# LuoweiZhou/VLP

Measured on NVIDIA H100. Metric: image_text_samples_per_sec, higher is better.
Workload: dtype bf16

## Files before the change

### include/vlpk.h

```cpp
#ifndef VLPK_H_
#define VLPK_H_

#include <stddef.h>
#include <stdint.h>

#ifdef __cplusplus
extern "C" {
#endif

#define VLPK_VERSION 102

#define VLPK_BF16 0
#define VLPK_F32 1
#define VLPK_I64 2
#define VLPK_MASK_ADDITIVE 0
#define VLPK_MASK_ZERO_ONE 1
#define VLPK_ACT_NONE 0
#define VLPK_ACT_RELU 1

typedef struct VlpkDropout {
  float p;
  uint64_t seed;
  const uint64_t* seed_dev;
} VlpkDropout;
// ... 105 lines not shown
                    int64_t k_bstride, const uint32_t* mask_bits, int mask_rows, int kv_slots, const float* lse, float* p, int64_t ld_p,
                    int64_t p_bstride, void* stream);

int vlpk_mha_fwd(const VlpkShape* s, const VlpkLayerWeights* w, const void* x, const void* x_kv, const uint32_t* mask_bits,
                 int mask_rows, VlpkLayerActs* a, float p_attn, float p_hidden, const VlpkDropout* drop, uint64_t layer_id,
                 void* stream);
int vlpk_ffn_fwd(const VlpkShape* s, const VlpkLayerWeights* w, VlpkLayerActs* a, float p_hidden, const VlpkDropout* drop,
                 uint64_t layer_id, void* stream);
int vlpk_layer_fwd(const VlpkShape* s, const VlpkLayerWeights* w, const void* x, const void* x_kv, const uint32_t* mask_bits,
                   int mask_rows, VlpkLayerActs* a, float p_attn, float p_hidden, const VlpkDropout* drop, uint64_t layer_id,
                   void* stream);
int vlpk_layer_bwd(const VlpkShape* s, const VlpkLayerWeights* w, const void* x, const uint32_t* mask_bits, int mask_rows,
                   const VlpkLayerActs* a, const void* dy, void* dx, const VlpkLayerGrads* g, const VlpkBwdScratch* ws,
                   float p_attn, float p_hidden, const VlpkDropout* drop, uint64_t layer_id, void* stream);

int vlpk_ffn_bwd(const VlpkShape* s, const VlpkLayerWeights* w, const VlpkLayerActs* a, const void* dy, void* dy1,
                 const VlpkLayerGrads* g, const VlpkBwdScratch* ws, float p_hidden, const VlpkDropout* drop, uint64_t layer_id,
                 void* stream);
int vlpk_mha_bwd(const VlpkShape* s, const VlpkLayerWeights* w, const void* x, const uint32_t* mask_bits, int mask_rows,
                 const VlpkLayerActs* a, const void* dy1, void* dx, const VlpkLayerGrads* g, const VlpkBwdScratch* ws, float p_attn,
                 float p_hidden, const VlpkDropout* drop, uint64_t layer_id, void* stream);
int vlpk_mha_incr_fwd(const VlpkShape* s, const VlpkLayerWeights* w, const void* x, const void* x_kv, const uint32_t* mask_bits,
                      int mask_rows, VlpkLayerActs* a, uint64_t layer_id, void* stream);
int vlpk_layer_cached_fwd(const VlpkShape* s, const VlpkLayerWeights* w, const void* x, void* kv_cache, int cache_rows, int pos,
                          const uint32_t* mask_bits, int mask_rows, VlpkLayerActs* a, uint64_t layer_id, void* stream);
int vlpk_layer_cached_group_fwd(const VlpkShape* s, const VlpkLayerWeights* w, const void* x, const void* prefix, int prefix_rows, int P,
                                void* text, int T, const int32_t* slots, int G, int pos, const uint32_t* mask_bits, int mask_rows,
                                VlpkLayerActs* a, uint64_t layer_id, void* stream);
int vlpk_workspace_bytes(const VlpkShape* s, size_t* out3);

int vlpk_encoder_fwd(const VlpkShape* s, int n_layers, const VlpkLayerWeights* w, const void* x, const uint32_t* mask_bits,
                     int mask_rows, VlpkLayerActs* acts, float p_attn, float p_hidden, const VlpkDropout* drop, void* stream);
int vlpk_encoder_bwd(const VlpkShape* s, int n_layers, const VlpkLayerWeights* w, const void* x, const uint32_t* mask_bits,
                     int mask_rows, const VlpkLayerActs* acts, const void* const* dys, void* dx0, const VlpkLayerGrads* grads,
                     const VlpkBwdScratch* ws, float p_attn, float p_hidden, const VlpkDropout* drop, void* stream);

int vlpk_decoder_ce_fwd(int R, int V, int H, const void* h, const void* w, const void* bias_pad, const int64_t* labels, void* logits,
                        float* lse, float* loss, void* stream);
int vlpk_decoder_ce_bwd(int R, int V, int H, const void* h, const void* w, const int64_t* labels, const void* logits, const float* lse,
                        const float* dloss, void* dlogits, float* dh, void* dw, float* dbias, void* stream);
int vlpk_decoder_ce_ls_fwd(int R, int V, int H, float eps, const void* h, const void* w, const void* bias_pad, const int64_t* labels,
                           void* logits, float* lse, float* loss, void* stream);
int vlpk_decoder_ce_ls_bwd(int R, int V, int H, float eps, const void* h, const void* w, const int64_t* labels, const void* logits,
                           const float* lse, const float* dloss, void* dlogits, float* dh, void* dw, float* dbias, void* stream);

typedef struct VlpkAdamTensor {
  void* param;
  const void* grad;
  float* master;
  float* m;
  float* v;
  int64_t n;
  float weight_decay;
  int32_t param_dtype;
  int32_t grad_dtype;
  int32_t reserved;
} VlpkAdamTensor;

int vlpk_bertadam_chunk(void);
int vlpk_bertadam_step(const VlpkAdamTensor* tensors_host, const VlpkAdamTensor* tensors_dev, const int32_t* chunk_prefix_host,
                       const int32_t* chunk_prefix_dev, int n_tensors, float* sqnorm_dev, double lr_scheduled, double b1, double b2,
                       double eps, double max_grad_norm, void* stream);

void vlpk_profile_enable(int on);
void vlpk_profile_reset(void);
int vlpk_profile_get(int cat, double* ms, double* work, int64_t* launches);
int64_t vlpk_launch_count(void);

int vlpk_beam_ngram_block(int rows, int K, int f, int T_cap, int n, const int32_t* hist_in, int32_t* hist_out, const int64_t* ptr,
                          const int64_t* wid, const int32_t* ignore, int n_ignore, float* logp, int64_t ld, int V, void* stream);

int vlpk_sample_tokens(int rows, int V, const void* logits, int64_t ld, const void* bias, int fp32, int mode, int topk, float topp,
                       uint64_t seed, int f, int64_t* seq, int T_cap, float* score, int32_t* finished, int32_t* live, int eos_id, int pad_id,
                       int block_eos, int n, const int32_t* ignore, int n_ignore, void* stream);

int vlpk_f32_to_bf16(const float* src, void* dst, int64_t n, void* stream);
int vlpk_colsum(const void* x, int64_t ld, int64_t M, int N, float* out, void* stream);
int vlpk_debug_dropout_mask(const VlpkDropout* drop, uint64_t site, int64_t n, unsigned char* out, void* stream);
int vlpk_add_bf16(void* dst, const void* a, const void* b, int64_t n, void* stream);

int vlpk_gemm(int M, int N, int K, int a_mn, const void* A, int64_t lda, int b_mn, const void* B, int64_t ldb, const void* bias,
              void* D0, int64_t ldd0, void* D1, int64_t ldd1, const void* aux, int64_t ld_aux, int epi, int splits, int bn,
              void* stream);

#ifdef __cplusplus
}
#endif
#endif
```

### vlp_b200/_lib.py

```python
import ctypes as C
import os

import torch

_HERE = os.path.dirname(os.path.abspath(__file__))
LIB_PATH = os.path.join(_HERE, "libvlpk.so")

c_void_p, c_int, c_i64, c_u64, c_float = C.c_void_p, C.c_int, C.c_int64, C.c_uint64, C.c_float


class VlpkDropout(C.Structure):
    _fields_ = [("p", c_float), ("seed", c_u64), ("seed_dev", c_void_p)]


class VlpkShape(C.Structure):
    _fields_ = [("B", C.c_int32), ("Lq", C.c_int32), ("Lkv", C.c_int32), ("H", C.c_int32), ("heads", C.c_int32),
                ("I", C.c_int32), ("kv_slots", C.c_int32)]


WEIGHT_FIELDS = ["wq", "wk", "wv", "bq", "bk", "bv", "wo", "bo", "ln1_g", "ln1_b", "w1", "b1", "w2", "b2", "ln2_g", "ln2_b"]
GRAD_FIELDS = ["wqkv", "bqkv", "wo", "bo", "ln1_g", "ln1_b", "w1", "b1", "w2", "b2", "ln2_g", "ln2_b"]
ACT_FIELDS = ["qkv", "ctx", "t1", "y1", "u", "hmid", "t2", "y", "lse", "stats1", "stats2", "kv", "drop_attn"]
SCRATCH_FIELDS = ["dz2", "dt2", "du", "dy1", "dz1", "dt1", "dctx", "dqkv", "dx"]

# ... 14 lines not shown
    _fields_ = [(n, c_void_p) for n in SCRATCH_FIELDS]


class VlpkAdamTensor(C.Structure):
    _fields_ = [("param", c_void_p), ("grad", c_void_p), ("master", c_void_p), ("m", c_void_p), ("v", c_void_p), ("n", c_i64),
                ("weight_decay", c_float), ("param_dtype", C.c_int32), ("grad_dtype", C.c_int32), ("reserved", C.c_int32)]


_P = c_void_p
_SIGS = {
    "vlpk_version": (c_int, []),
    "vlpk_last_error": (C.c_char_p, []),
    "vlpk_debug_set_option": (c_int, [C.c_char_p, c_int]),
    "vlpk_set_reserved_sms": (None, [c_int]),
    "vlpk_set_deterministic": (None, [c_int]),
    "vlpk_debug_plan_gemm": (c_int, [c_int] * 10 + [C.POINTER(c_int)]),
    "vlpk_mask_pack": (c_int, [_P, c_int, c_int, c_int, c_int, c_int, c_i64, c_i64, _P, _P]),
    "vlpk_mask_synth": (c_int, [_P, _P, c_int, c_int, c_int, _P, _P]),
    "vlpk_linear_fwd": (c_int, [c_int, c_int, c_int, _P, c_i64, _P, c_i64, _P, _P, c_i64, c_int, C.POINTER(VlpkDropout), c_u64, _P]),
    "vlpk_linear_bwd": (c_int, [c_int, c_int, c_int, _P, c_i64, _P, c_i64, _P, c_i64, _P, c_i64, _P, _P, c_i64, _P, c_i64, _P,
                                c_int, c_float, _P]),
    "vlpk_embed_fwd": (c_int, [c_int, c_int, c_int, c_int, c_int, _P, _P, _P, _P, _P, _P, _P, _P, _P, _P, _P, _P,
                               C.POINTER(VlpkDropout), c_u64, _P]),
    "vlpk_embed_bwd": (c_int, [c_int, c_int, c_int, c_int, c_int, _P, _P, _P, _P, _P, _P, _P, _P, _P, _P, _P, _P, _P, _P,
                               C.POINTER(VlpkDropout), c_u64, _P]),
    "vlpk_embed_tables_bwd": (c_int, [c_int, c_int, c_int, c_int, c_int, _P, _P, _P, _P, c_int, c_int, c_int, _P, _P, _P, _P, _P]),
    "vlpk_ln_res_drop_fwd": (c_int, [c_i64, c_int, _P, _P, _P, _P, _P, _P, C.POINTER(VlpkDropout), c_u64, _P]),
    "vlpk_ln_res_drop_bwd": (c_int, [c_i64, c_int, _P, _P, _P, _P, _P, _P, _P, _P, _P, _P, C.POINTER(VlpkDropout), c_u64, _P]),
    "vlpk_attn_core_fwd": (c_int, [c_int, c_int, c_int, c_int, _P, c_i64, _P, _P, c_i64, _P, c_int, _P, c_i64, _P,
                                   C.POINTER(VlpkDropout), c_u64, _P]),
    "vlpk_attn_core_bwd": (c_int, [c_int, c_int, c_int, _P, _P, _P, c_i64, _P, c_int, _P, _P, c_i64, _P, _P, _P, _P, c_i64,
                                   C.POINTER(VlpkDropout), c_u64, _P]),
    "vlpk_attn_core_fwd_wide": (c_int, [c_int, c_int, c_int, c_int, _P, c_i64, _P, _P, c_i64, _P, c_int, _P, c_i64, _P,
                                        C.POINTER(VlpkDropout), c_u64, c_int, _P]),
    "vlpk_attn_core_bwd_wide": (c_int, [c_int, c_int, c_int, _P, _P, _P, c_i64, _P, c_int, _P, _P, c_i64, _P, _P, _P, _P, c_i64,
                                        C.POINTER(VlpkDropout), c_u64, c_int, _P]),
    "vlpk_attn_probs": (c_int, [c_int, c_int, c_int, c_int, c_int, _P, c_i64, c_i64, _P, c_i64, c_i64, _P, c_int, c_int, _P, _P, c_i64,
                                c_i64, _P]),
    "vlpk_mha_fwd": (c_int, [C.POINTER(VlpkShape), C.POINTER(VlpkLayerWeights), _P, _P, _P, c_int, C.POINTER(VlpkLayerActs),
                             c_float, c_float, C.POINTER(VlpkDropout), c_u64, _P]),
    "vlpk_ffn_fwd": (c_int, [C.POINTER(VlpkShape), C.POINTER(VlpkLayerWeights), C.POINTER(VlpkLayerActs), c_float,
                             C.POINTER(VlpkDropout), c_u64, _P]),
    "vlpk_layer_fwd": (c_int, [C.POINTER(VlpkShape), C.POINTER(VlpkLayerWeights), _P, _P, _P, c_int, C.POINTER(VlpkLayerActs),
                               c_float, c_float, C.POINTER(VlpkDropout), c_u64, _P]),
    "vlpk_layer_bwd": (c_int, [C.POINTER(VlpkShape), C.POINTER(VlpkLayerWeights), _P, _P, c_int, C.POINTER(VlpkLayerActs), _P, _P,
                               C.POINTER(VlpkLayerGrads), C.POINTER(VlpkBwdScratch), c_float, c_float, C.POINTER(VlpkDropout),
                               c_u64, _P]),
    "vlpk_ffn_bwd": (c_int, [C.POINTER(VlpkShape), C.POINTER(VlpkLayerWeights), C.POINTER(VlpkLayerActs), _P, _P,
                             C.POINTER(VlpkLayerGrads), C.POINTER(VlpkBwdScratch), c_float, C.POINTER(VlpkDropout), c_u64, _P]),
    "vlpk_mha_bwd": (c_int, [C.POINTER(VlpkShape), C.POINTER(VlpkLayerWeights), _P, _P, c_int, C.POINTER(VlpkLayerActs), _P, _P,
                             C.POINTER(VlpkLayerGrads), C.POINTER(VlpkBwdScratch), c_float, c_float, C.POINTER(VlpkDropout),
                             c_u64, _P]),
    "vlpk_mha_incr_fwd": (c_int, [C.POINTER(VlpkShape), C.POINTER(VlpkLayerWeights), _P, _P, _P, c_int,
                                  C.POINTER(VlpkLayerActs), c_u64, _P]),
    "vlpk_layer_cached_fwd": (c_int, [C.POINTER(VlpkShape), C.POINTER(VlpkLayerWeights), _P, _P, c_int, c_int, _P, c_int,
                                      C.POINTER(VlpkLayerActs), c_u64, _P]),
    "vlpk_layer_cached_group_fwd": (c_int, [C.POINTER(VlpkShape), C.POINTER(VlpkLayerWeights), _P, _P, c_int, c_int, _P, c_int, _P, c_int,
                                            c_int, _P, c_int, C.POINTER(VlpkLayerActs), c_u64, _P]),
    "vlpk_workspace_bytes": (c_int, [C.POINTER(VlpkShape), C.POINTER(C.c_size_t)]),
    "vlpk_encoder_fwd": (c_int, [C.POINTER(VlpkShape), c_int, C.POINTER(VlpkLayerWeights), _P, _P, c_int,
                                 C.POINTER(VlpkLayerActs), c_float, c_float, C.POINTER(VlpkDropout), _P]),
    "vlpk_encoder_bwd": (c_int, [C.POINTER(VlpkShape), c_int, C.POINTER(VlpkLayerWeights), _P, _P, c_int,
                                 C.POINTER(VlpkLayerActs), C.POINTER(c_void_p), _P, C.POINTER(VlpkLayerGrads),
                                 C.POINTER(VlpkBwdScratch), c_float, c_float, C.POINTER(VlpkDropout), _P]),
    "vlpk_decoder_ce_fwd": (c_int, [c_int, c_int, c_int, _P, _P, _P, _P, _P, _P, _P, _P]),
    "vlpk_decoder_ce_bwd": (c_int, [c_int, c_int, c_int, _P, _P, _P, _P, _P, _P, _P, _P, _P, _P, _P]),
    "vlpk_decoder_ce_ls_fwd": (c_int, [c_int, c_int, c_int, c_float, _P, _P, _P, _P, _P, _P, _P, _P]),
    "vlpk_decoder_ce_ls_bwd": (c_int, [c_int, c_int, c_int, c_float, _P, _P, _P, _P, _P, _P, _P, _P, _P, _P, _P]),
    "vlpk_bertadam_chunk": (c_int, []),
    "vlpk_bertadam_step": (c_int, [_P, _P, _P, _P, c_int, _P, C.c_double, C.c_double, C.c_double, C.c_double, C.c_double, _P]),
    "vlpk_profile_enable": (None, [c_int]),
    "vlpk_profile_reset": (None, []),
    "vlpk_profile_get": (c_int, [c_int, C.POINTER(C.c_double), C.POINTER(C.c_double), C.POINTER(c_i64)]),
    "vlpk_launch_count": (c_i64, []),
    "vlpk_beam_ngram_block": (c_int, [c_int, c_int, c_int, c_int, c_int, _P, _P, _P, _P, _P, c_int, _P, c_i64, c_int, _P]),
    "vlpk_sample_tokens": (c_int, [c_int, c_int, _P, c_i64, _P, c_int, c_int, c_int, c_float, c_u64, c_int, _P, c_int, _P, _P, _P, c_int,
                                   c_int, c_int, c_int, _P, c_int, _P]),
    "vlpk_f32_to_bf16": (c_int, [_P, _P, c_i64, _P]),
    "vlpk_colsum": (c_int, [_P, c_i64, c_i64, c_int, _P, _P]),
    "vlpk_debug_dropout_mask": (c_int, [C.POINTER(VlpkDropout), c_u64, c_i64, _P, _P]),
    "vlpk_add_bf16": (c_int, [_P, _P, _P, c_i64, _P]),
    "vlpk_gemm": (c_int, [c_int, c_int, c_int, c_int, _P, c_i64, c_int, _P, c_i64, _P, _P, c_i64, _P, c_i64, _P, c_i64, c_int,
                          c_int, c_int, _P]),
}
EXPORTED_SYMBOLS = tuple(_SIGS.keys())

_lib = None


def lib():
    global _lib
    if _lib is None:
        if not os.path.exists(LIB_PATH):
            raise RuntimeError(
                f"{LIB_PATH} not found: build it with `python -c 'import __graft_entry__ as g; g.build()'` "
                "(vlp_b200 has no CPU / PyTorch fallback path)")
        l = C.CDLL(LIB_PATH)
        for name, (res, args) in _SIGS.items():
            fn = getattr(l, name)
            fn.restype = res
            fn.argtypes = args
        _lib = l
    return _lib


def check(rc, what):
    if rc != 0:
        msg = lib().vlpk_last_error()
        raise RuntimeError(f"{what} failed (rc={rc}): {msg.decode() if msg else '?'}")


def ptr(t):
    return None if t is None else t.data_ptr()


def stream():
    return torch.cuda.current_stream().cuda_stream


_deterministic = False


def call(name, *args):
    global _deterministic
    det = torch.are_deterministic_algorithms_enabled()
    if det != _deterministic:
        invoke("vlpk_set_deterministic", int(det))
        _deterministic = det
    invoke(name, *args)


def invoke(name, *args):
    rc = getattr(lib(), name)(*args)
    if rc is not None:
        check(rc, name)
```

### vlp_b200/csrc/api.cu

```cuda
#include "../../include/vlpk.h"

#include <cstdlib>
#include <cstring>

#include "attn.cuh"
#include "decode.cuh"
#include "gemm.cuh"
#include "head.cuh"
#include "host.cuh"
#include "optim.cuh"
#include "rowops.cuh"
#include "tables.cuh"

using namespace vlpk;
typedef __nv_bfloat16 bf16;

namespace {

inline cudaStream_t S(void* s) { return reinterpret_cast<cudaStream_t>(s); }

enum { SITE_ATTN = 0, SITE_HID1 = 1, SITE_HID2 = 2 };
inline uint64_t site_of(uint64_t layer_id, int site) { return layer_id * 8 + site; }

inline DropoutCfg mk_drop(const VlpkDropout* d, float p, uint64_t site) {
// ... 718 lines not shown
                           const float* lse, const float* dloss, void* dlogits, float* dh, void* dw, float* dbias, void* stream) {
  VLPK_CHECK_ARG(eps > 0.f && eps <= 1.f && V >= 3, "decoder_ce_ls: label smoothing %g with V=%d (needs 0 < eps <= 1, V >= 3)",
                 static_cast<double>(eps), V);
  DecoderCeArgs a;
  a.R = R; a.V = V; a.H = H; a.eps = eps;
  a.h = h; a.w = w;
  a.labels = reinterpret_cast<const long long*>(labels);
  a.logits = const_cast<void*>(logits);
  a.lse = const_cast<float*>(lse);
  a.dloss = dloss; a.dlogits = dlogits; a.dh = dh; a.dw = dw; a.dbias = dbias;
  return launch_decoder_ce_bwd(a, S(stream));
}

int vlpk_bertadam_chunk(void) { return ADAM_CHUNK; }

int vlpk_bertadam_step(const VlpkAdamTensor* tensors_host, const VlpkAdamTensor* tensors_dev, const int32_t* chunk_prefix_host,
                       const int32_t* chunk_prefix_dev, int n_tensors, float* sqnorm_dev, double lr_scheduled, double b1, double b2,
                       double eps, double max_grad_norm, void* stream) {
  VLPK_CHECK_ARG(b1 >= 0.0 && b1 < 1.0 && b2 >= 0.0 && b2 < 1.0 && eps >= 0.0, "bertadam: b1=%g b2=%g eps=%g out of range", b1, b2, eps);
  AdamHyper h;
  h.lr = static_cast<float>(lr_scheduled);
  h.b1 = static_cast<float>(b1); h.omb1 = static_cast<float>(1.0 - b1);
  h.b2 = static_cast<float>(b2); h.omb2 = static_cast<float>(1.0 - b2);
  h.eps = static_cast<float>(eps);
  h.max_grad_norm = static_cast<float>(max_grad_norm);
  return launch_bertadam(tensors_host, tensors_dev, chunk_prefix_host, chunk_prefix_dev, n_tensors, sqnorm_dev, h, S(stream));
}

void vlpk_profile_enable(int on) { prof_enable(on != 0); }
void vlpk_profile_reset(void) { prof_reset(); }
int vlpk_profile_get(int cat, double* ms, double* work, int64_t* launches) {
  long long n = 0;
  const int rc = prof_get(cat, ms, work, &n);
  *launches = n;
  return rc;
}
int64_t vlpk_launch_count(void) { return launch_count(); }

int vlpk_f32_to_bf16(const float* src, void* dst, int64_t n, void* stream) { return launch_f32_to_bf16(src, dst, n, S(stream)); }

int vlpk_debug_dropout_mask(const VlpkDropout* drop, uint64_t site, int64_t n, unsigned char* out, void* stream) {
  VLPK_CHECK_ARG(drop != nullptr && out != nullptr, "dropout_mask: null pointer");
  return launch_dropout_mask(mk_drop(drop, drop->p, site), n, out, S(stream));
}

int vlpk_beam_ngram_block(int rows, int K, int f, int T_cap, int n, const int32_t* hist_in, int32_t* hist_out, const int64_t* ptr,
                          const int64_t* wid, const int32_t* ignore, int n_ignore, float* logp, int64_t ld, int V, void* stream) {
  NgramBlockArgs a;
  a.rows = rows; a.K = K; a.f = f; a.T_cap = T_cap; a.n = n;
  a.hist_in = hist_in; a.hist_out = hist_out;
  a.ptr = reinterpret_cast<const long long*>(ptr); a.wid = reinterpret_cast<const long long*>(wid);
  a.ignore = ignore; a.n_ignore = n_ignore;
  a.logp = logp; a.ld = ld; a.V = V;
  return launch_beam_ngram_block(a, S(stream));
}

int vlpk_sample_tokens(int rows, int V, const void* logits, int64_t ld, const void* bias, int fp32, int mode, int topk, float topp,
                       uint64_t seed, int f, int64_t* seq, int T_cap, float* score, int32_t* finished, int32_t* live, int eos_id, int pad_id,
                       int block_eos, int n, const int32_t* ignore, int n_ignore, void* stream) {
  SampleArgs a;
  a.rows = rows; a.V = V; a.logits = logits; a.ld = ld; a.bias = bias; a.fp32 = fp32;
  a.mode = mode; a.topk = topk; a.topp = topp; a.seed = seed;
  a.f = f; a.seq = reinterpret_cast<long long*>(seq); a.T_cap = T_cap; a.score = score;
  a.finished = finished; a.live = live; a.eos_id = eos_id; a.pad_id = pad_id; a.block_eos = block_eos;
  a.n = n; a.ignore = ignore; a.n_ignore = n_ignore;
  return launch_sample(a, S(stream));
}

int vlpk_colsum(const void* x, int64_t ld, int64_t M, int N, float* out, void* stream) {
  VLPK_CHECK_ARG(x && out, "colsum: null pointer");
  return launch_colsum(x, ld, M, N, out, S(stream));
}

int vlpk_add_bf16(void* dst, const void* a, const void* b, int64_t n, void* stream) {
  VLPK_CHECK_ARG(dst && a && b, "add_bf16: null pointer");
  if (n <= 0) return 0;
  LaunchScope scope(CAT_MISC, 6.0 * n, S(stream));
  add_bf16_kernel<<<static_cast<unsigned>(((n + 7) / 8 + 255) / 256), 256, 0, S(stream)>>>(static_cast<bf16*>(dst), static_cast<const bf16*>(a),
                                                                                        static_cast<const bf16*>(b), n);
  VLPK_CUDA(cudaGetLastError());
  return 0;
}

int vlpk_gemm(int M, int N, int K, int a_mn, const void* A, int64_t lda, int b_mn, const void* B, int64_t ldb, const void* bias, void* D0,
              int64_t ldd0, void* D1, int64_t ldd1, const void* aux, int64_t ld_aux, int epi, int splits, int bn, void* stream) {
  VLPK_CHECK_ARG(A && B && D0, "gemm: null pointer");
  GemmDesc g;
  g.M = M; g.N = N; g.K = K;
  g.a_mn = a_mn != 0; g.A = A; g.lda = lda;
  g.b_mn = b_mn != 0; g.B[0] = B; g.ldb = ldb; g.nseg = 1;
  g.bias[0] = static_cast<const bf16*>(bias);
  g.D0 = D0; g.ldd0 = ldd0; g.D1 = D1; g.ldd1 = ldd1;
  g.aux = static_cast<const bf16*>(aux); g.ld_aux = ld_aux;
  g.epi = epi; g.splits = splits; g.bn = bn;
  if (deterministic() && epi == EPI_REDUCE_F32) return launch_gemm_split_slices(g, SCRATCH_SPLITK, S(stream));
  return launch_gemm(g, S(stream));
}

}
#pragma GCC visibility pop
```

### vlp_b200/csrc/gemm.cu

```cuda
#include "gemm.cuh"

#include <cstdlib>

#include "host.cuh"
#include "rowops.cuh"

namespace vlpk {

static constexpr int BM = 128;
static constexpr int BK = 64;
static constexpr int NUM_THREADS = 384;
static constexpr int PRODUCER_REGS = 24;
static constexpr int CONSUMER_REGS = 240;
static constexpr int STG_BYTES = 64 * 128;
static constexpr int STG_PER_CONSUMER = 4;
static constexpr int SMEM_MAX = 232448;
static constexpr int BN = 128;

struct GemmTmaps {
  CUtensorMap a;
  CUtensorMap b[3];
  CUtensorMap d0;
  CUtensorMap d1;
  CUtensorMap aux;
};

struct GemmArgs {
  int M, N, K;
  int b_seg_rows;
  int splits;
  int split_slices;
  const __nv_bfloat16* bias[3];
  float relu_scale;
  DropoutCfg drop;
  float* colsum;
};

template <int STAGES>
struct SmemLayout {
  static constexpr int A_BYTES = BM * BK * 2;
  static constexpr int B_BYTES = BN * BK * 2;
  static constexpr int STAGE_BYTES = A_BYTES + B_BYTES;
  static constexpr int OFF_STG = STAGES * STAGE_BYTES;
  static constexpr int OFF_BAR = OFF_STG + 2 * STG_PER_CONSUMER * STG_BYTES;
  static constexpr int NUM_BARS = 3 * STAGES + 2;
  static constexpr int TOTAL = OFF_BAR + NUM_BARS * 8;
  static constexpr int DYN_BYTES = TOTAL + 1024;
  static_assert(DYN_BYTES <= SMEM_MAX, "shared memory budget exceeded");
};

struct StageCount {
  static constexpr int value = (SMEM_MAX - 1024 - 2 * STG_PER_CONSUMER * STG_BYTES - 256) / (BM * BK * 2 + BN * BK * 2);
};

__device__ __forceinline__ void wg_bar_sync(int cw) {
  asm volatile("bar.sync %0, 128;" ::"r"(cw + 1) : "memory");
}

template <bool A_MN, bool B_MN, int EPI>
__global__ void __launch_bounds__(NUM_THREADS, 1)
gemm_kernel(const __grid_constant__ GemmTmaps tm, const GemmArgs args) {
  constexpr int STAGES = StageCount::value;
  using L = SmemLayout<STAGES>;
  extern __shared__ uint8_t smem_raw[];
  uint8_t* smem = reinterpret_cast<uint8_t*>((reinterpret_cast<uintptr_t>(smem_raw) + 1023) & ~uintptr_t(1023));

  uint64_t* bars = reinterpret_cast<uint64_t*>(smem + L::OFF_BAR);
  uint64_t* full_bar = bars;
  uint64_t* empty_bar = bars + 2 * STAGES;
  uint64_t* aux_bar = bars + 3 * STAGES;
  constexpr bool HAS_AUX = (EPI == EPI_ADD || EPI == EPI_MUL || EPI == EPI_DRELU);

  pdl_launch_dependents();
  const int wg = __shfl_sync(0xffffffffu, threadIdx.x >> 7, 0);
  const int lane = threadIdx.x & 31;

  const int num_m = (args.M + BM - 1) / BM;
  const int num_n = (args.N + BN - 1) / BN;
  const int total_kb = (args.K + BK - 1) / BK;
  const int kb_per = (total_kb + args.splits - 1) / args.splits;
  const int num_work = num_m * num_n * args.splits;

  if (threadIdx.x == 0) {
    tma_prefetch_desc(&tm.a);
    tma_prefetch_desc(&tm.b[0]);
    tma_prefetch_desc(&tm.d0);
    if (HAS_AUX) tma_prefetch_desc(&tm.aux);
    for (int i = 0; i < 2 * STAGES; ++i) mbar_init(&full_bar[i], 1);
    for (int i = 0; i < STAGES; ++i) mbar_init(&empty_bar[i], 4);
    for (int i = 0; i < 2; ++i) mbar_init(&aux_bar[i], 1);
    fence_mbar_init();
  }
  __syncthreads();
  pdl_wait();

  if (wg == 0) {
    setmaxnreg_dec<PRODUCER_REGS>();
    if (threadIdx.x < 32) {
      int stage = 0;
      uint32_t phase = 0;
      int item = 0;
      for (int w = blockIdx.x; w < num_work; w += gridDim.x, ++item) {
        uint64_t* fb = full_bar + (item & 1) * STAGES;
        const int n_blk = w % num_n;
        const int m_blk = (w / num_n) % num_m;
        const int split = w / (num_n * num_m);
        const int kb0 = split * kb_per;
        const int kb1 = min(total_kb, kb0 + kb_per);
        const int m0 = m_blk * BM;
        for (int kb = kb0; kb < kb1; ++kb) {
          mbar_wait(&empty_bar[stage], phase ^ 1u);
          if (elect_one()) {
            uint8_t* sA = smem + stage * L::STAGE_BYTES;
            uint8_t* sB = sA + L::A_BYTES;
            mbar_arrive_expect_tx(&fb[stage], L::STAGE_BYTES);
            if (!A_MN) {
              tma_load_2d(sA, &tm.a, &fb[stage], kb * BK, m0);
            } else {
#pragma unroll
              for (int j = 0; j < BM / 64; ++j) tma_load_2d(sA + j * 8192, &tm.a, &fb[stage], m0 + j * 64, kb * BK);
            }
            if (!B_MN) {
              const int n0 = n_blk * BN;
              const int seg = n0 / args.b_seg_rows;
              tma_load_2d(sB, &tm.b[seg], &fb[stage], kb * BK, n0 - seg * args.b_seg_rows);
            } else {
              const int k0 = kb * BK;
              const int seg = k0 / args.b_seg_rows;
#pragma unroll
              for (int j = 0; j < BN / 64; ++j)
                tma_load_2d(sB + j * 8192, &tm.b[seg], &fb[stage], n_blk * BN + j * 64, k0 - seg * args.b_seg_rows);
            }
          }
          __syncwarp();
          if (++stage == STAGES) {
            stage = 0;
            phase ^= 1u;
          }
        }
      }
    }
  } else {
    setmaxnreg_inc<CONSUMER_REGS>();
    const int cw = wg - 1;
    const int t = threadIdx.x - 128 * wg;
    const int fr = (t >> 5) * 16 + (lane >> 2);
    const int fc = (lane & 3) * 2;
    const bool store_thread = (t == 0);
    const uint64_t dseed = drop_seed(args.drop);
    constexpr bool HAS_BIAS = !B_MN && (EPI == EPI_STORE || EPI == EPI_GELU || EPI == EPI_RELU);
    uint8_t* stg_base = smem + L::OFF_STG + cw * STG_PER_CONSUMER * STG_BYTES;
    const uint32_t a_base = smem_u32(smem);
    const uint32_t b_base = smem_u32(smem) + L::A_BYTES;
    uint64_t* fb = full_bar + cw * STAGES;
    int stage = 0;
    uint32_t phases = 0;
    uint32_t box_seq = 0;
    uint32_t aux_phase = 0;
    bool timed_out = false;
    float acc[2][BN / 2];
#pragma unroll
    for (int i = 0; i < BN / 2; ++i) acc[0][i] = acc[1][i] = 0.f;
    for (int w = blockIdx.x + cw * gridDim.x; w < num_work; w += 2 * gridDim.x) {
      const int w_other = w - static_cast<int>(gridDim.x);
      if (w_other >= static_cast<int>(blockIdx.x)) {
        const int split_o = w_other / (num_n * num_m);
        const int kb0_o = split_o * kb_per;
        stage = (stage + min(total_kb, kb0_o + kb_per) - kb0_o) % STAGES;
      }
      const int n_blk = w % num_n;
      const int m_blk = (w / num_n) % num_m;
      const int split = w / (num_n * num_m);
      const int kb0 = split * kb_per;
      const int kb1 = min(total_kb, kb0 + kb_per);
      const int n0 = n_blk * BN;

      int prev_stage = 0;
      for (int kb = kb0; kb < kb1; ++kb) {
        mbar_wait_flag(&fb[stage], (phases >> stage) & 1u, timed_out);
        phases ^= 1u << stage;
        const uint32_t sa = a_base + stage * L::STAGE_BYTES;
        const uint32_t sb = b_base + stage * L::STAGE_BYTES;
        reg_fence(acc[0]);
        reg_fence(acc[1]);
        wgmma_fence();
#pragma unroll
        for (int k = 0; k < BK / 16; ++k) {
          const uint64_t bdesc = B_MN ? wgmma_desc_sw128(sb + k * 2048, 8192, 1024) : wgmma_desc_sw128(sb + k * 32, 16, 1024);
#pragma unroll
          for (int h = 0; h < 2; ++h) {
            const uint32_t sah = sa + h * 8192;
            const uint64_t adesc = A_MN ? wgmma_desc_sw128(sah + k * 2048, 8192, 1024) : wgmma_desc_sw128(sah + k * 32, 16, 1024);
            wgmma_m64n128k16_ss<A_MN ? 1 : 0, B_MN ? 1 : 0>(acc[h], adesc, bdesc, (kb > kb0 || k > 0) ? 1u : 0u);
          }
        }
        wgmma_commit();
        if (HAS_AUX && kb == kb0) {
          static_assert(STG_PER_CONSUMER == 2 * (BN / 64), "one staging box per aux box of a tile");
          wg_bar_sync(cw);
          if (store_thread) {
            tma_store_wait_read<0>();
            fence_proxy_async_smem();
            mbar_arrive_expect_tx(&aux_bar[cw], STG_PER_CONSUMER * STG_BYTES);
#pragma unroll
            for (int b = 0; b < STG_PER_CONSUMER; ++b)
              tma_load_2d(stg_base + b * STG_BYTES, &tm.aux, &aux_bar[cw], n0 + (b & 1) * 64, m_blk * BM + (b >> 1) * 64);
          }
        }
        wgmma_wait<1>();
        reg_fence(acc[0]);
        reg_fence(acc[1]);
        if (kb > kb0 && lane == 0) mbar_arrive(&empty_bar[prev_stage]);
        prev_stage = stage;
        if (++stage == STAGES) stage = 0;
      }
      wgmma_wait<0>();
      reg_fence(acc[0]);
      reg_fence(acc[1]);
      if (lane == 0) mbar_arrive(&empty_bar[prev_stage]);

      if (EPI == EPI_REDUCE_F32) {
        constexpr int NBOX = BN / 32;
#pragma unroll
        for (int h = 0; h < 2; ++h) {
          const int m0 = m_blk * BM + h * 64;
#pragma unroll
          for (int c = 0; c < NBOX; ++c) {
            uint8_t* stg = stg_base + (box_seq % STG_PER_CONSUMER) * STG_BYTES;
            if (store_thread) tma_store_wait_read<STG_PER_CONSUMER - 1>();
            wg_bar_sync(cw);
#pragma unroll
            for (int j = 0; j < 8; ++j) {
              const int i = c * 16 + 2 * j;
              const int r = fr + 8 * (j & 1), col = 8 * (j >> 1) + fc;
              *reinterpret_cast<float2*>(stg + r * 128 + (((col >> 2) ^ (r & 7)) << 4) + (col & 3) * 4) = make_float2(acc[h][i], acc[h][i + 1]);
            }
            fence_proxy_async_smem();
            wg_bar_sync(cw);
            if (store_thread) {
              tma_reduce_add_3d(&tm.d0, stg, n0 + c * 32, m0, args.split_slices ? split : 0);
              tma_store_commit();
            }
            ++box_seq;
          }
        }
      } else {
        constexpr int NBOX = BN / 64;
        if (HAS_AUX) {
          mbar_wait_flag(&aux_bar[cw], aux_phase, timed_out);
          aux_phase ^= 1u;
        }
        const __nv_bfloat16* bp = nullptr;
        int bias_off = 0;
        if (HAS_BIAS) {
          const int seg = n0 / args.b_seg_rows;
          bp = args.bias[seg];
          bias_off = seg * args.b_seg_rows;
        }
#pragma unroll
        for (int h = 0; h < 2; ++h) {
          const int m0 = m_blk * BM + h * 64;
          int nh = n0;
          const __nv_bfloat16* bph = bp;
          uint64_t dsh = dseed;
          asm volatile("" : "+r"(nh), "+l"(bph), "+l"(dsh));
#pragma unroll
          for (int c = 0; c < NBOX; ++c) {
            uint8_t* stg = (EPI == EPI_GELU) ? stg_base + (box_seq & 1u) * 2 * STG_BYTES : stg_base + (box_seq % STG_PER_CONSUMER) * STG_BYTES;
            uint8_t* stg_g = stg + STG_BYTES;
            if (store_thread) {
              if (EPI == EPI_GELU) tma_store_wait_read<STG_PER_CONSUMER / 2 - 1>(); else tma_store_wait_read<STG_PER_CONSUMER - 1>();
            }
            wg_bar_sync(cw);
#pragma unroll
            for (int j = 0; j < 16; ++j) {
              const int i = c * 32 + 2 * j;
              const int r = fr + 8 * (j & 1), col = 8 * (j >> 1) + fc;
              const int n = nh + c * 64 + col;
              const long long m = m0 + r;
              const int so = r * 128 + (((col >> 3) ^ (r & 7)) << 4) + (col & 7) * 2;
              float v0 = acc[h][i], v1 = acc[h][i + 1];
              if (HAS_BIAS) {
                if (bph != nullptr && n < args.N) {
                  const float2 bb = unpack_bf16x2(__ldg(reinterpret_cast<const unsigned int*>(bph + n - bias_off)));
                  v0 += bb.x;
                  v1 += bb.y;
                }
              }
              if (EPI == EPI_GELU) {
                float g0, d0, g1, d1;
                gelu_and_grad(v0, g0, d0);
                gelu_and_grad(v1, g1, d1);
                *reinterpret_cast<uint32_t*>(stg + so) = pack_bf16x2(d0, d1);
                *reinterpret_cast<uint32_t*>(stg_g + so) = pack_bf16x2(g0, g1);
                continue;
              }
              if (EPI == EPI_RELU) {
                uint32_t keep = 0xFFu;
                if (args.drop.p > 0.f)
                  keep = dropout_keep8(dsh, args.drop.site, (static_cast<uint64_t>(m) * args.N + (n - fc)) >> 3, args.drop.thresh16);
                v0 = fmaxf(v0, 0.f);
                v1 = fmaxf(v1, 0.f);
                v0 = ((keep >> fc) & 1u) ? v0 * args.drop.scale : 0.f;
                v1 = ((keep >> (fc + 1)) & 1u) ? v1 * args.drop.scale : 0.f;
              } else if (EPI == EPI_ADD || EPI == EPI_MUL || EPI == EPI_DRELU) {
                const float2 x = unpack_bf16x2(*reinterpret_cast<const uint32_t*>(stg + so));
                if (EPI == EPI_ADD) {
                  v0 += x.x;
                  v1 += x.y;
                } else if (EPI == EPI_MUL) {
                  v0 *= x.x;
                  v1 *= x.y;
                } else {
                  v0 = x.x > 0.f ? v0 * args.relu_scale : 0.f;
                  v1 = x.y > 0.f ? v1 * args.relu_scale : 0.f;
                }
              }
              *reinterpret_cast<uint32_t*>(stg + so) = pack_bf16x2(v0, v1);
            }
            fence_proxy_async_smem();
            wg_bar_sync(cw);
            if (store_thread) {
              tma_store_2d(&tm.d0, stg, nh + c * 64, m0);
              if (EPI == EPI_GELU) tma_store_2d(&tm.d1, stg_g, nh + c * 64, m0);
              tma_store_commit();
            }
            if (EPI != EPI_GELU && args.colsum != nullptr) {
              const int col = t & 63, r0 = (t >> 6) * 32;
              float acc_c = 0.f;
#pragma unroll 8
              for (int rr = r0; rr < r0 + 32; ++rr) {
                const __nv_bfloat16 v = *reinterpret_cast<const __nv_bfloat16*>(stg + rr * 128 + (((col >> 3) ^ (rr & 7)) << 4) + (col & 7) * 2);
                acc_c += __bfloat162float(v);
              }
              if (nh + c * 64 + col < args.N) atomicAdd(args.colsum + nh + c * 64 + col, acc_c);
            }
            ++box_seq;
          }
        }
      }
    }
    if (store_thread) tma_store_wait<0>();
    if (timed_out) __trap();
  }
}

template <bool A_MN, bool B_MN, int EPI>
static int launch_inst(const GemmTmaps& tm, const GemmArgs& args, int num_work, cudaStream_t stream) {
  constexpr int STAGES = StageCount::value;
  using L = SmemLayout<STAGES>;
  auto kfn = gemm_kernel<A_MN, B_MN, EPI>;
  static bool attr_set = false;
  if (!attr_set) {
    VLPK_CUDA(cudaFuncSetAttribute(kfn, cudaFuncAttributeMaxDynamicSharedMemorySize, L::DYN_BYTES));
    attr_set = true;
  }
  const int max_ctas = gemm_sms();
  const int ctas = num_work < max_ctas ? num_work : max_ctas;
  LaunchScope scope(A_MN ? CAT_GEMM_WGRAD : (B_MN ? CAT_GEMM_DGRAD : CAT_GEMM_FWD), 2.0 * args.M * args.N * args.K, stream);
  VLPK_CUDA(launch_ex(kfn, dim3(ctas), dim3(NUM_THREADS), L::DYN_BYTES, stream, 1, tm, args));
  return 0;
}

static int dispatch(const GemmDesc& g, const GemmTmaps& tm, const GemmArgs& args, int num_work, cudaStream_t s) {
  if (!g.a_mn && !g.b_mn) {
    switch (g.epi) {
      case EPI_STORE: return launch_inst<false, false, EPI_STORE>(tm, args, num_work, s);
      case EPI_GELU: return launch_inst<false, false, EPI_GELU>(tm, args, num_work, s);
      case EPI_RELU: return launch_inst<false, false, EPI_RELU>(tm, args, num_work, s);
      default: break;
    }
  } else if (!g.a_mn && g.b_mn) {
    switch (g.epi) {
      case EPI_STORE: return launch_inst<false, true, EPI_STORE>(tm, args, num_work, s);
      case EPI_ADD: return launch_inst<false, true, EPI_ADD>(tm, args, num_work, s);
      case EPI_MUL: return launch_inst<false, true, EPI_MUL>(tm, args, num_work, s);
      case EPI_DRELU: return launch_inst<false, true, EPI_DRELU>(tm, args, num_work, s);
      case EPI_REDUCE_F32: return launch_inst<false, true, EPI_REDUCE_F32>(tm, args, num_work, s);
      default: break;
    }
  } else if (g.a_mn && g.b_mn) {
    if (g.epi == EPI_REDUCE_F32) return launch_inst<true, true, EPI_REDUCE_F32>(tm, args, num_work, s);
    if (g.epi == EPI_STORE) return launch_inst<true, true, EPI_STORE>(tm, args, num_work, s);
  }
  set_error("gemm: unsupported (a_mn=%d, b_mn=%d, epi=%d) combination", (int)g.a_mn, (int)g.b_mn, g.epi);
  return -1;
}

static double tile_cost(int M, int N, int total_kb, int splits, bool reduce) {
  const int num_m = (M + BM - 1) / BM;
  const int num_n = (N + BN - 1) / BN;
  const long long tiles = static_cast<long long>(num_m) * num_n * splits;
  const int slots = deterministic() ? num_sms() : gemm_sms();
  const long long rounds = (tiles + slots - 1) / slots;
  const int kb_per = (total_kb + splits - 1) / splits;
  const double mainloop = kb_per * (128.0 + double(BN));
  const double epi = (reduce ? 3.0 : 1.5) * BN;
  return rounds * (mainloop + epi + 60.0);
}

int plan_gemm(const GemmDesc& g, int* bn_out, int* splits_out) {
  const int seg_rows = g.nseg > 1 ? g.b_seg_rows : (g.b_mn ? g.K : g.N);
  const int total_kb = (g.K + BK - 1) / BK;
  const bool reduce = (g.epi == EPI_REDUCE_F32);
  VLPK_CHECK_ARG(g.bn == 0 || g.bn == BN, "gemm: no valid tile configuration (bn=%d; tiles are %d wide)", g.bn, BN);
  VLPK_CHECK_ARG(g.nseg == 1 || seg_rows % (g.b_mn ? BK : BN) == 0, "gemm: segment rows %d not tile aligned", seg_rows);
  int splits = 1;
  if (reduce) {
    const int max_s = total_kb / 8 > 0 ? total_kb / 8 : 1;
    if (g.splits > 0) {
      splits = g.splits < max_s ? g.splits : max_s;
    } else {
      double best = 1e300;
      for (int s = 1; s <= max_s; ++s) {
        const double c = tile_cost(g.M, g.N, total_kb, s, reduce);
        if (c < best) {
          best = c;
          splits = s;
        }
      }
    }
  }
  if (splits > total_kb) splits = total_kb;
  {
    const int kb_per = (total_kb + splits - 1) / splits;
    splits = (total_kb + kb_per - 1) / kb_per;
  }
  *bn_out = BN;
  *splits_out = splits;
  return 0;
}

int launch_gemm(const GemmDesc& g, cudaStream_t stream) {
  VLPK_CHECK_ARG(g.M > 0 && g.N > 0 && g.K > 0, "gemm: empty problem M=%d N=%d K=%d", g.M, g.N, g.K);
  VLPK_CHECK_ARG(g.N % 8 == 0, "gemm: N=%d must be a multiple of 8", g.N);
  VLPK_CHECK_ARG(g.nseg >= 1 && g.nseg <= 3, "gemm: nseg=%d", g.nseg);
  const int seg_rows = g.nseg > 1 ? g.b_seg_rows : (g.b_mn ? g.K : g.N);
  const bool reduce = (g.epi == EPI_REDUCE_F32);
  VLPK_CHECK_ARG(g.splits <= 1 || reduce, "gemm: split-K needs EPI_REDUCE_F32");
  VLPK_CHECK_ARG(g.b_rows == 0 || (g.nseg == 1 && g.b_rows <= (g.b_mn ? g.K : g.N)), "gemm: b_rows=%d needs a single B segment", g.b_rows);

  int bn = BN, splits = 1;
  VLPK_TRY(plan_gemm(g, &bn, &splits));

  GemmTmaps tm;
  memset(&tm, 0, sizeof(tm));
  if (!g.a_mn) {
    VLPK_TRY(make_tmap_2d(&tm.a, TM_BF16, g.A, g.K, g.M, g.lda, BK, BM));
  } else {
    VLPK_TRY(make_tmap_2d(&tm.a, TM_BF16, g.A, g.M, g.K, g.lda, 64, BK));
  }
  for (int s = 0; s < g.nseg; ++s) {
    if (!g.b_mn) {
      const int rows = g.nseg > 1 ? seg_rows : (g.b_rows > 0 ? g.b_rows : g.N);
      VLPK_TRY(make_tmap_2d(&tm.b[s], TM_BF16, g.B[s], g.K, rows, g.ldb, BK, bn));
    } else {
      const int rows = g.nseg > 1 ? seg_rows : (g.b_rows > 0 ? g.b_rows : g.K);
      VLPK_TRY(make_tmap_2d(&tm.b[s], TM_BF16, g.B[s], g.N, rows, g.ldb, 64, BK));
    }
  }
  for (int s = g.nseg; s < 3; ++s) tm.b[s] = tm.b[0];
  if (reduce) {
    VLPK_CHECK_ARG(g.split_stride == 0 || (g.split_stride % 4 == 0 && g.split_stride >= static_cast<int64_t>(g.M) * g.ldd0),
                   "gemm: split_stride %lld must be a multiple of 4 and cover M x ldd0", (long long)g.split_stride);
    const uint64_t dims[3] = {static_cast<uint64_t>(g.N), static_cast<uint64_t>(g.M), static_cast<uint64_t>(g.split_stride ? splits : 1)};
    const uint64_t strides[2] = {static_cast<uint64_t>(g.ldd0) * 4,
                                 static_cast<uint64_t>(g.split_stride ? g.split_stride : static_cast<int64_t>(g.M) * g.ldd0) * 4};
    const uint32_t box[3] = {32, 64, 1};
    VLPK_TRY(make_tmap(&tm.d0, TM_F32, 3, g.D0, dims, strides, box));
    tm.d1 = tm.d0;
  } else {
    VLPK_TRY(make_tmap_2d(&tm.d0, TM_BF16, g.D0, g.N, g.M, g.ldd0, 64, 64));
    if (g.epi == EPI_GELU) {
      VLPK_CHECK_ARG(g.D1 != nullptr, "gemm: EPI_GELU needs D1");
      VLPK_TRY(make_tmap_2d(&tm.d1, TM_BF16, g.D1, g.N, g.M, g.ldd1, 64, 64));
    } else {
      tm.d1 = tm.d0;
    }
  }
  VLPK_CHECK_ARG(g.colsum == nullptr || (!reduce && g.epi != EPI_GELU), "gemm: colsum fusion is for single-output bf16 epilogues");
  if (g.epi == EPI_ADD || g.epi == EPI_MUL || g.epi == EPI_DRELU) {
    VLPK_CHECK_ARG(g.aux != nullptr && (g.ld_aux % 8) == 0 && (reinterpret_cast<uintptr_t>(g.aux) & 15u) == 0,
                   "gemm: aux must be 16-byte aligned with ld %% 8 == 0");
    VLPK_TRY(make_tmap_2d(&tm.aux, TM_BF16, g.aux, g.N, g.M, g.ld_aux, 64, 64));
  } else {
    tm.aux = tm.d0;
  }

  GemmArgs a;
  a.M = g.M;
  a.N = g.N;
  a.K = g.K;
  a.b_seg_rows = seg_rows;
  a.splits = splits;
  a.split_slices = (reduce && g.split_stride > 0) ? 1 : 0;
  for (int s = 0; s < 3; ++s) a.bias[s] = (s < g.nseg) ? g.bias[s] : nullptr;
  a.relu_scale = g.relu_scale;
  a.colsum = g.colsum;
  a.drop = g.drop;

  const int num_m = (g.M + BM - 1) / BM;
  const int num_n = (g.N + bn - 1) / bn;
  const int num_work = num_m * num_n * splits;
  return dispatch(g, tm, a, num_work, stream);
}

int launch_gemm_split_slices(GemmDesc g, int slot, cudaStream_t stream) {
  VLPK_CHECK_ARG(g.epi == EPI_REDUCE_F32 && g.split_stride == 0, "gemm: split slices are for EPI_REDUCE_F32 into one D0");
  int bn = 0, splits = 1;
  VLPK_TRY(plan_gemm(g, &bn, &splits));
  if (splits == 1) return launch_gemm(g, stream);
  VLPK_CHECK_ARG(g.ldd0 == g.N, "gemm: split slices need a dense D0 (ldd0 %lld != N %d)", (long long)g.ldd0, g.N);
  const long long n = static_cast<long long>(g.M) * g.N;
  float* part = scratch_f32(slot, static_cast<size_t>(n) * splits, stream);
  if (part == nullptr) return -1;
  VLPK_CUDA(cudaMemsetAsync(part, 0, static_cast<size_t>(n) * splits * sizeof(float), stream));
  float* out = static_cast<float*>(g.D0);
  g.D0 = part;
  g.splits = splits;
  g.split_stride = n;
  VLPK_TRY(launch_gemm(g, stream));
  return launch_sum_parts(part, splits, n, out, stream);
}

}
```

Measured before the change: 5411.

## Stage bias and colsum in shared memory vectors within GEMM epilogue

Each consumer warpgroup now loads its tile's bias once into a small shared-memory vector and reuses it in the epilogue, replacing repeated global bias loads per element. Aux values are read from staging into registers ahead of the loop, and one warpgroup barrier on the aux path is removed. Column sums are computed from the packed outputs in registers with warp shuffles, reduced through shared-memory atomics, and written with one global atomic per column per tile instead of per 32-row box. This uses extra shared memory, which may lower the pipeline stage count, and adds a debug entry point that exposes the colsum argument.

```diff
diff --git a/include/vlpk.h b/include/vlpk.h
--- a/include/vlpk.h
+++ b/include/vlpk.h
@@ -211,6 +211,9 @@
 int vlpk_gemm(int M, int N, int K, int a_mn, const void* A, int64_t lda, int b_mn, const void* B, int64_t ldb, const void* bias,
               void* D0, int64_t ldd0, void* D1, int64_t ldd1, const void* aux, int64_t ld_aux, int epi, int splits, int bn,
               void* stream);
+int vlpk_debug_gemm_colsum(int M, int N, int K, int a_mn, const void* A, int64_t lda, int b_mn, const void* B, int64_t ldb,
+                           const void* bias, void* D0, int64_t ldd0, void* D1, int64_t ldd1, const void* aux, int64_t ld_aux, int epi,
+                           int splits, int bn, float* colsum, void* stream);
 
 #ifdef __cplusplus
 }
diff --git a/vlp_b200/_lib.py b/vlp_b200/_lib.py
--- a/vlp_b200/_lib.py
+++ b/vlp_b200/_lib.py
@@ -120,6 +120,8 @@
     "vlpk_add_bf16": (c_int, [_P, _P, _P, c_i64, _P]),
     "vlpk_gemm": (c_int, [c_int, c_int, c_int, c_int, _P, c_i64, c_int, _P, c_i64, _P, _P, c_i64, _P, c_i64, _P, c_i64, c_int,
                           c_int, c_int, _P]),
+    "vlpk_debug_gemm_colsum": (c_int, [c_int, c_int, c_int, c_int, _P, c_i64, c_int, _P, c_i64, _P, _P, c_i64, _P, c_i64, _P, c_i64,
+                                       c_int, c_int, c_int, _P, _P]),
 }
 EXPORTED_SYMBOLS = tuple(_SIGS.keys())
 
diff --git a/vlp_b200/csrc/api.cu b/vlp_b200/csrc/api.cu
--- a/vlp_b200/csrc/api.cu
+++ b/vlp_b200/csrc/api.cu
@@ -824,8 +824,9 @@
   return 0;
 }
 
-int vlpk_gemm(int M, int N, int K, int a_mn, const void* A, int64_t lda, int b_mn, const void* B, int64_t ldb, const void* bias, void* D0,
-              int64_t ldd0, void* D1, int64_t ldd1, const void* aux, int64_t ld_aux, int epi, int splits, int bn, void* stream) {
+int vlpk_debug_gemm_colsum(int M, int N, int K, int a_mn, const void* A, int64_t lda, int b_mn, const void* B, int64_t ldb,
+                           const void* bias, void* D0, int64_t ldd0, void* D1, int64_t ldd1, const void* aux, int64_t ld_aux, int epi,
+                           int splits, int bn, float* colsum, void* stream) {
   VLPK_CHECK_ARG(A && B && D0, "gemm: null pointer");
   GemmDesc g;
   g.M = M; g.N = N; g.K = K;
@@ -835,9 +836,16 @@
   g.D0 = D0; g.ldd0 = ldd0; g.D1 = D1; g.ldd1 = ldd1;
   g.aux = static_cast<const bf16*>(aux); g.ld_aux = ld_aux;
   g.epi = epi; g.splits = splits; g.bn = bn;
+  g.colsum = colsum;
   if (deterministic() && epi == EPI_REDUCE_F32) return launch_gemm_split_slices(g, SCRATCH_SPLITK, S(stream));
   return launch_gemm(g, S(stream));
 }
 
+int vlpk_gemm(int M, int N, int K, int a_mn, const void* A, int64_t lda, int b_mn, const void* B, int64_t ldb, const void* bias, void* D0,
+              int64_t ldd0, void* D1, int64_t ldd1, const void* aux, int64_t ld_aux, int epi, int splits, int bn, void* stream) {
+  return vlpk_debug_gemm_colsum(M, N, K, a_mn, A, lda, b_mn, B, ldb, bias, D0, ldd0, D1, ldd1, aux, ld_aux, epi, splits, bn, nullptr,
+                                stream);
+}
+
 }
 #pragma GCC visibility pop
diff --git a/vlp_b200/csrc/gemm.cu b/vlp_b200/csrc/gemm.cu
--- a/vlp_b200/csrc/gemm.cu
+++ b/vlp_b200/csrc/gemm.cu
@@ -16,6 +16,7 @@
 static constexpr int STG_PER_CONSUMER = 4;
 static constexpr int SMEM_MAX = 232448;
 static constexpr int BN = 128;
+static constexpr int VEC_BYTES = BN * 4;
 
 struct GemmTmaps {
   CUtensorMap a;
@@ -42,7 +43,8 @@
   static constexpr int B_BYTES = BN * BK * 2;
   static constexpr int STAGE_BYTES = A_BYTES + B_BYTES;
   static constexpr int OFF_STG = STAGES * STAGE_BYTES;
-  static constexpr int OFF_BAR = OFF_STG + 2 * STG_PER_CONSUMER * STG_BYTES;
+  static constexpr int OFF_VEC = OFF_STG + 2 * STG_PER_CONSUMER * STG_BYTES;
+  static constexpr int OFF_BAR = OFF_VEC + 2 * VEC_BYTES;
   static constexpr int NUM_BARS = 3 * STAGES + 2;
   static constexpr int TOTAL = OFF_BAR + NUM_BARS * 8;
   static constexpr int DYN_BYTES = TOTAL + 1024;
@@ -50,11 +52,22 @@
 };
 
 struct StageCount {
-  static constexpr int value = (SMEM_MAX - 1024 - 2 * STG_PER_CONSUMER * STG_BYTES - 256) / (BM * BK * 2 + BN * BK * 2);
+  static constexpr int value =
+      (SMEM_MAX - 1024 - 2 * STG_PER_CONSUMER * STG_BYTES - 2 * VEC_BYTES - 256) / (BM * BK * 2 + BN * BK * 2);
 };
 
 __device__ __forceinline__ void wg_bar_sync(int cw) {
   asm volatile("bar.sync %0, 128;" ::"r"(cw + 1) : "memory");
+}
+
+template <int W>
+__device__ __forceinline__ void fold_lanes(float* s, int lane) {
+  const bool upper = (lane & W) != 0;
+#pragma unroll
+  for (int i = 0; i < W / 2; ++i) {
+    const float lo = s[i], hi = s[i + W / 2];
+    s[i] = (upper ? hi : lo) + __shfl_xor_sync(0xffffffffu, upper ? lo : hi, W);
+  }
 }
 
 template <bool A_MN, bool B_MN, int EPI>
@@ -150,6 +163,8 @@
     const uint64_t dseed = drop_seed(args.drop);
     constexpr bool HAS_BIAS = !B_MN && (EPI == EPI_STORE || EPI == EPI_GELU || EPI == EPI_RELU);
     uint8_t* stg_base = smem + L::OFF_STG + cw * STG_PER_CONSUMER * STG_BYTES;
+    float* vec = reinterpret_cast<float*>(smem + L::OFF_VEC + cw * VEC_BYTES);
+    vec[t] = 0.f;
     const uint32_t a_base = smem_u32(smem);
     const uint32_t b_base = smem_u32(smem) + L::A_BYTES;
     uint64_t* fb = full_bar + cw * STAGES;
@@ -176,6 +191,7 @@
       const int n0 = n_blk * BN;
 
       int prev_stage = 0;
+      float bias_t = 0.f;
       for (int kb = kb0; kb < kb1; ++kb) {
         mbar_wait_flag(&fb[stage], (phases >> stage) & 1u, timed_out);
         phases ^= 1u << stage;
@@ -195,9 +211,13 @@
           }
         }
         wgmma_commit();
+        if (HAS_BIAS && kb == kb0) {
+          const int seg = n0 / args.b_seg_rows;
+          const __nv_bfloat16* bp = args.bias[seg];
+          if (bp != nullptr && n0 + t < args.N) bias_t = __bfloat162float(__ldg(bp + n0 + t - seg * args.b_seg_rows));
+        }
         if (HAS_AUX && kb == kb0) {
           static_assert(STG_PER_CONSUMER == 2 * (BN / 64), "one staging box per aux box of a tile");
-          wg_bar_sync(cw);
           if (store_thread) {
             tma_store_wait_read<0>();
             fence_proxy_async_smem();
@@ -218,6 +238,7 @@
       reg_fence(acc[0]);
       reg_fence(acc[1]);
       if (lane == 0) mbar_arrive(&empty_bar[prev_stage]);
+      if (HAS_BIAS) vec[t] = bias_t;
 
       if (EPI == EPI_REDUCE_F32) {
         constexpr int NBOX = BN / 32;
@@ -250,20 +271,15 @@
           mbar_wait_flag(&aux_bar[cw], aux_phase, timed_out);
           aux_phase ^= 1u;
         }
-        const __nv_bfloat16* bp = nullptr;
-        int bias_off = 0;
-        if (HAS_BIAS) {
-          const int seg = n0 / args.b_seg_rows;
-          bp = args.bias[seg];
-          bias_off = seg * args.b_seg_rows;
-        }
+        const bool has_bias = HAS_BIAS && args.bias[n0 / args.b_seg_rows] != nullptr;
+        const bool has_colsum = !HAS_BIAS && EPI != EPI_GELU && args.colsum != nullptr;
+        float cs[NBOX][2] = {};
 #pragma unroll
         for (int h = 0; h < 2; ++h) {
           const int m0 = m_blk * BM + h * 64;
           int nh = n0;
-          const __nv_bfloat16* bph = bp;
           uint64_t dsh = dseed;
-          asm volatile("" : "+r"(nh), "+l"(bph), "+l"(dsh));
+          asm volatile("" : "+r"(nh), "+l"(dsh));
 #pragma unroll
           for (int c = 0; c < NBOX; ++c) {
             uint8_t* stg = (EPI == EPI_GELU) ? stg_base + (box_seq & 1u) * 2 * STG_BYTES : stg_base + (box_seq % STG_PER_CONSUMER) * STG_BYTES;
@@ -272,6 +288,16 @@
               if (EPI == EPI_GELU) tma_store_wait_read<STG_PER_CONSUMER / 2 - 1>(); else tma_store_wait_read<STG_PER_CONSUMER - 1>();
             }
             wg_bar_sync(cw);
+            uint32_t out[16];
+            constexpr bool BIAS_REGS = HAS_BIAS && EPI != EPI_RELU;
+            float2 bias2[8];
+            uint32_t aux2[16];
+#pragma unroll
+            for (int j = 0; j < 16; ++j) {
+              const int r = fr + 8 * (j & 1), col = 8 * (j >> 1) + fc;
+              if (BIAS_REGS && (j & 1) == 0) bias2[j >> 1] = *reinterpret_cast<const float2*>(vec + c * 64 + col);
+              if (HAS_AUX) aux2[j] = *reinterpret_cast<const uint32_t*>(stg + r * 128 + (((col >> 3) ^ (r & 7)) << 4) + (col & 7) * 2);
+            }
 #pragma unroll
             for (int j = 0; j < 16; ++j) {
               const int i = c * 32 + 2 * j;
@@ -280,12 +306,10 @@
               const long long m = m0 + r;
               const int so = r * 128 + (((col >> 3) ^ (r & 7)) << 4) + (col & 7) * 2;
               float v0 = acc[h][i], v1 = acc[h][i + 1];
-              if (HAS_BIAS) {
-                if (bph != nullptr && n < args.N) {
-                  const float2 bb = unpack_bf16x2(__ldg(reinterpret_cast<const unsigned int*>(bph + n - bias_off)));
-                  v0 += bb.x;
-                  v1 += bb.y;
-                }
+              if (has_bias) {
+                const float2 bb = BIAS_REGS ? bias2[j >> 1] : *reinterpret_cast<const float2*>(vec + c * 64 + col);
+                v0 += bb.x;
+                v1 += bb.y;
               }
               if (EPI == EPI_GELU) {
                 float g0, d0, g1, d1;
@@ -304,7 +328,7 @@
                 v0 = ((keep >> fc) & 1u) ? v0 * args.drop.scale : 0.f;
                 v1 = ((keep >> (fc + 1)) & 1u) ? v1 * args.drop.scale : 0.f;
               } else if (EPI == EPI_ADD || EPI == EPI_MUL || EPI == EPI_DRELU) {
-                const float2 x = unpack_bf16x2(*reinterpret_cast<const uint32_t*>(stg + so));
+                const float2 x = unpack_bf16x2(aux2[j]);
                 if (EPI == EPI_ADD) {
                   v0 += x.x;
                   v1 += x.y;
@@ -316,7 +340,8 @@
                   v1 = x.y > 0.f ? v1 * args.relu_scale : 0.f;
                 }
               }
-              *reinterpret_cast<uint32_t*>(stg + so) = pack_bf16x2(v0, v1);
+              out[j] = pack_bf16x2(v0, v1);
+              *reinterpret_cast<uint32_t*>(stg + so) = out[j];
             }
             fence_proxy_async_smem();
             wg_bar_sync(cw);
@@ -325,18 +350,35 @@
               if (EPI == EPI_GELU) tma_store_2d(&tm.d1, stg_g, nh + c * 64, m0);
               tma_store_commit();
             }
-            if (EPI != EPI_GELU && args.colsum != nullptr) {
-              const int col = t & 63, r0 = (t >> 6) * 32;
-              float acc_c = 0.f;
-#pragma unroll 8
-              for (int rr = r0; rr < r0 + 32; ++rr) {
-                const __nv_bfloat16 v = *reinterpret_cast<const __nv_bfloat16*>(stg + rr * 128 + (((col >> 3) ^ (rr & 7)) << 4) + (col & 7) * 2);
-                acc_c += __bfloat162float(v);
+            if (EPI != EPI_GELU && has_colsum) {
+              float s[16];
+#pragma unroll
+              for (int q = 0; q < 8; ++q) {
+                const float2 a = unpack_bf16x2(out[2 * q]), b = unpack_bf16x2(out[2 * q + 1]);
+                s[2 * q] = a.x + b.x;
+                s[2 * q + 1] = a.y + b.y;
               }
-              if (nh + c * 64 + col < args.N) atomicAdd(args.colsum + nh + c * 64 + col, acc_c);
+              fold_lanes<16>(s, lane);
+              fold_lanes<8>(s, lane);
+              fold_lanes<4>(s, lane);
+              cs[c][0] += s[0];
+              cs[c][1] += s[1];
             }
             ++box_seq;
           }
+        }
+        if (EPI != EPI_GELU && has_colsum) {
+          const int q = ((lane >> 4) & 1) * 4 + ((lane >> 3) & 1) * 2 + ((lane >> 2) & 1);
+#pragma unroll
+          for (int c = 0; c < NBOX; ++c) {
+#pragma unroll
+            for (int e = 0; e < 2; ++e)
+              asm volatile("red.shared.add.f32 [%0], %1;" ::"r"(smem_u32(vec + c * 64 + 8 * q + fc + e)), "f"(cs[c][e]) : "memory");
+          }
+          wg_bar_sync(cw);
+          const float v = vec[t];
+          vec[t] = 0.f;
+          if (n0 + t < args.N) atomicAdd(args.colsum + n0 + t, v);
         }
       }
     }
@@ -478,7 +520,8 @@
       tm.d1 = tm.d0;
     }
   }
-  VLPK_CHECK_ARG(g.colsum == nullptr || (!reduce && g.epi != EPI_GELU), "gemm: colsum fusion is for single-output bf16 epilogues");
+  VLPK_CHECK_ARG(g.colsum == nullptr || (!reduce && g.epi != EPI_GELU && g.b_mn),
+                 "gemm: colsum fusion is for single-output bf16 dgrad epilogues");
   if (g.epi == EPI_ADD || g.epi == EPI_MUL || g.epi == EPI_DRELU) {
     VLPK_CHECK_ARG(g.aux != nullptr && (g.ld_aux % 8) == 0 && (reinterpret_cast<uintptr_t>(g.aux) & 15u) == 0,
                    "gemm: aux must be 16-byte aligned with ld %% 8 == 0");
```

Result: faster. 5484 (median of 6 runs) (+1.3%).
